# anuragranj/cc

Measured on AMD Instinct MI355X. Metric: train images/sec (832x256, 5-frame sample, 6-scale CC step), higher is better.
Workload: dtype f32; 1 GPU; full CC: DispResNet6+PoseNetB6+MaskNet6+Back2Future, all losses; per_gpu_batch=4, global_batch=4, height=256, width=832, scales=6, frames=5, parallelism=dp1, hipgraph=True, trained_nets=all, rccl_ranks=1, dead_occlusion_decoders_elided=False, net_streams=2, pipeline=per_network, grad_chunks=False, deterministic=True

## Files before the change

### cc_amd/csrc/wgrad_thin.hip

```cpp
#include <stdio.h>
#include <type_traits>
#include <stdlib.h>
#include "cc_common.h"
#include "conv_internal.h"
#include "cc_tools.h"

namespace {

typedef float f32x4 __attribute__((ext_vector_type(4)));

constexpr int THIN_NW = 4;

struct WT {
    const float* a; const float* x; float* ws;
    int B, M, AH, AW; long a_bs;
    int Cin, IH, IW; long x_bs;
    int R, nxc, units, upb, npb, ngc, ngt, swz;
};

template <int S, int SI, int PAD, int TR>
struct ThinCfg {
    static constexpr int PQ = (PAD + 3) / 4;
    static constexpr int IMAX = SI * 3 + S - 1 - PAD + 4 * PQ;
    static constexpr int NQ = IMAX / 4 + 1;
    static constexpr int TS = TR * S;
};

template <int S, int SI, int PAD, int TR, int DBG>
__device__ __forceinline__ void wgrad_thin_body(const WT& g, const int bx_, const int by_) {
    typedef ThinCfg<S, SI, PAD, TR> C;
    constexpr int PQ = C::PQ, NQ = C::NQ, TS = C::TS;
    __shared__ float red[TS * 256];
    const int lane = threadIdx.x & 63;
    const int wave = __builtin_amdgcn_readfirstlane((int)(threadIdx.x >> 6));
    const int i = lane & 15, k = lane >> 4;
    int combo = by_;
    const int tg = combo % g.ngt;
    combo /= g.ngt;
    const int cg = combo % g.ngc, mg = combo / g.ngc;
    const int r0 = tg * TR;
    const int m = mg * 16 + i, c = cg * 16 + i;
    const bool mok = m < g.M, cok = c < g.Cin;
    const float* __restrict__ abase = g.a + (long)(mok ? m : 0) * g.AH * g.AW;
    const float* __restrict__ xbase = g.x + (long)(cok ? c : 0) * g.IH * g.IW;

    f32x4 acc[TR][S];
#pragma unroll
    for (int tr = 0; tr < TR; tr++)
#pragma unroll
        for (int s = 0; s < S; s++) acc[tr][s] = (f32x4){0.f, 0.f, 0.f, 0.f};

    const int pb = (g.swz ? ((bx_ & 7) * (g.npb >> 3) + (bx_ >> 3)) : bx_);
    const int u0 = pb * g.upb;
    const int u1 = (u0 + g.upb < g.units) ? (u0 + g.upb) : g.units;

    constexpr int KEEP = (TR > SI) ? TR - SI : 0;
    float4 An;
    float4 Wn[TR][NQ], Wc[TR][NQ];
    auto issue = [&](auto T0, int b, int y, int xc, float4& A, float4 (&W)[TR][NQ]) {
        constexpr int t0 = decltype(T0)::value;
        const int x0 = xc * 16 + 4 * k;
        const int xa = (x0 < g.AW) ? x0 : 0;
        A = *(const float4*)(abase + (unsigned)(b * (int)g.a_bs + y * g.AW + xa));
        const unsigned xb = (unsigned)(b * (int)g.x_bs);
#pragma unroll
        for (int tr = t0; tr < TR; tr++) {
            int iy = y * SI + r0 + tr - PAD;
            iy = iy < 0 ? 0 : (iy >= g.IH ? g.IH - 1 : iy);
            const unsigned xr = xb + (unsigned)(iy * g.IW);
#pragma unroll
            for (int q = 0; q < NQ; q++) {
                int col = SI * x0 - 4 * PQ + 4 * q;
                col = (col < 0 || col >= g.IW) ? 0 : col;
                W[tr][q] = *(const float4*)(xbase + (xr + (unsigned)col));
            }
        }
    };

    const int ngx = (g.nxc + THIN_NW - 1) / THIN_NW;
    int u = u0;
    const int ue = u1;
    if (u < ue) {
        int nb, ny, nxcpos;
        {
            const int colu = u / g.AH;
            ny = u - colu * g.AH;
            nb = colu / ngx;
            nxcpos = (colu - nb * ngx) * THIN_NW + wave;
        }
        typedef std::integral_constant<int, 0> ALL;
        typedef std::integral_constant<int, KEEP> NEW;
        issue(ALL(), nb, ny, nxcpos, An, Wn);
        bool fresh = true;
        for (; u < ue; u++) {
            const float4 Ac = An;
            if (fresh) {
#pragma unroll
                for (int tr = 0; tr < TR; tr++)
#pragma unroll
                    for (int q = 0; q < NQ; q++) Wc[tr][q] = Wn[tr][q];
            } else {
#pragma unroll
                for (int tr = 0; tr < TR; tr++)
#pragma unroll
                    for (int q = 0; q < NQ; q++) Wc[tr][q] = (tr < KEEP) ? Wc[tr + (TR - KEEP)][q] : Wn[tr][q];
            }
            const int y = ny, xc = nxcpos;
            if (u + 1 < ue) {
                fresh = false;
                if (++ny == g.AH) {
                    ny = 0;
                    fresh = true;
                    nxcpos += THIN_NW;
                    if (nxcpos - wave >= g.nxc) { nxcpos = wave; nb++; }
                }
                if (DBG != 2) {
                    if (fresh) issue(ALL(), nb, ny, nxcpos, An, Wn);
                    else issue(NEW(), nb, ny, nxcpos, An, Wn);
                }
            }

            const int x0 = xc * 16 + 4 * k;
            const bool aok = mok && (x0 < g.AW);
            float a4[4];
            a4[0] = aok ? Ac.x : 0.f;
            a4[1] = aok ? Ac.y : 0.f;
            a4[2] = aok ? Ac.z : 0.f;
            a4[3] = aok ? Ac.w : 0.f;
#pragma unroll
            for (int tr = 0; tr < TR; tr++) {
                const int iy = y * SI + r0 + tr - PAD;
                const bool rok = cok && (r0 + tr < g.R) && iy >= 0 && iy < g.IH;
                float w[NQ * 4];
#pragma unroll
                for (int q = 0; q < NQ; q++) {
                    const int col = SI * x0 - 4 * PQ + 4 * q;
                    const bool ok = rok && col >= 0 && col < g.IW;
                    w[4 * q + 0] = ok ? Wc[tr][q].x : 0.f;
                    w[4 * q + 1] = ok ? Wc[tr][q].y : 0.f;
                    w[4 * q + 2] = ok ? Wc[tr][q].z : 0.f;
                    w[4 * q + 3] = ok ? Wc[tr][q].w : 0.f;
                }
                if (DBG == 1) {
#pragma unroll
                    for (int s = 0; s < S; s++)
#pragma unroll
                        for (int j = 0; j < 4; j++) acc[tr][s][j] += a4[j] * w[SI * j + s - PAD + 4 * PQ];
                    continue;
                }
#pragma unroll
                for (int j = 0; j < 4; j++)
#pragma unroll
                    for (int s = 0; s < S; s++)
                        acc[tr][s] = __builtin_amdgcn_mfma_f32_16x16x4f32(a4[j], w[SI * j + s - PAD + 4 * PQ], acc[tr][s], 0, 0, 0);
            }
        }
    }

#pragma unroll 1
    for (int wv = 0; wv < THIN_NW; wv++) {
        if (wave == wv) {
#pragma unroll
            for (int tr = 0; tr < TR; tr++)
#pragma unroll
                for (int s = 0; s < S; s++)
#pragma unroll
                    for (int r = 0; r < 4; r++) {
                        const int idx = ((tr * S + s) * 4 + r) * 64 + lane;
                        const float v = acc[tr][s][r];
                        red[idx] = (wv == 0) ? v : (red[idx] + v);
                    }
        }
        __syncthreads();
    }
    float* __restrict__ slab = g.ws + ((long)by_ * g.npb + pb) * (TS * 256);
    for (int e = threadIdx.x; e < TS * 256; e += 64 * THIN_NW) {
        const int t = e >> 8, mc = e & 255, mm = mc >> 4, cc_ = mc & 15;
        slab[e] = red[(t * 4 + (mm & 3)) * 64 + (mm >> 2) * 16 + cc_];
    }
}


template <int S, int SI, int PAD, int TR, int DBG = 0>
__global__ __launch_bounds__(64 * THIN_NW) void k_wgrad_thin(WT g) {
    wgrad_thin_body<S, SI, PAD, TR, DBG>(g, (int)blockIdx.x, (int)blockIdx.y);
}

constexpr int THIN_MAXP = 24;
struct WTM { WT p[THIN_MAXP]; int blk_end[THIN_MAXP]; int n; };
template <int S, int SI, int PAD, int TR>
__global__ __launch_bounds__(64 * THIN_NW) void k_wgrad_thin_multi(WTM a) {
    int k = 0, first = 0;
#pragma unroll 1
    for (int q = 0; q + 1 < a.n; q++)
        if ((int)blockIdx.x >= a.blk_end[q]) { k = q + 1; first = a.blk_end[q]; }
#if defined(__HIP_DEVICE_COMPILE__) && !defined(CC_HIPEMU)
    const WT& g = *(reinterpret_cast<const WT*>((const char*)__builtin_amdgcn_kernarg_segment_ptr() + offsetof(WTM, p)) + k);
#else
    const WT& g = a.p[k];
#endif
    const int b = (int)blockIdx.x - first;
    const int by = b / g.npb;
    wgrad_thin_body<S, SI, PAD, TR, 0>(g, b - by * g.npb, by);
}


int env_int(const char* name, int dflt) { return cctools::env_int(name, dflt); }

struct ThinPlan {
    bool ok;
    int kind, TR, ngm, ngc, ngt, nxc, units, upb, npb, TS;
    size_t ws_floats;
};

enum { K_3_1 = 0, K_3_2, K_7_2, K_7_1, K_1_1, K_5_2, K_4_2, K_1_2, K_NONE };

ThinPlan plan_thin(int B, int M, int AH, int AW, int Cin, int R, int S, int si) {
    ThinPlan p = {};
    p.kind = K_NONE;
    if (R != S || env_int("CC_NO_WGRAD_THIN", 0)) return p;
    if (S == 3 && si == 1) { p.kind = K_3_1; p.TR = 3; }
    else if (S == 3 && si == 2) { p.kind = K_3_2; p.TR = 3; }
    else if (S == 7 && si == 2) { p.kind = K_7_2; p.TR = 2; }
    else if (S == 7 && si == 1) { p.kind = K_7_1; p.TR = 2; }
    else if (S == 1 && si == 1) { p.kind = K_1_1; p.TR = 1; }
    else if (S == 5 && si == 2) { p.kind = K_5_2; p.TR = 3; }
    else if (S == 4 && si == 2) { p.kind = K_4_2; p.TR = 4; }
    else if (S == 1 && si == 2) { p.kind = K_1_2; p.TR = 1; }
    else return p;
    p.ngm = (M + 15) / 16;
    p.ngc = (Cin + 15) / 16;
    const long P = (long)B * AH * AW;
    if ((AW & 3) || p.ngm * p.ngc > env_int("CC_WGRAD_THIN_MAXCOMBO", 15) || P < env_int("CC_WGRAD_THIN_MINPIX", 8192) ||
        (S == 7 && Cin < 8)) return p;
    p.ngt = (R + p.TR - 1) / p.TR;
    p.TS = p.TR * S;
    p.nxc = (AW + 15) / 16;
    const long units = (long)B * AH * ((p.nxc + THIN_NW - 1) / THIN_NW);
    if (units > (1l << 30)) return p;
    p.units = (int)units;
    long npb = units / env_int("CC_WGRAD_THIN_UPB", 8);
    const long cap = env_int("CC_WGRAD_THIN_NPB", 256);
    npb = npb < 1 ? 1 : (npb > cap ? cap : npb);
    p.upb = (int)((units + npb - 1) / npb);
    p.npb = (p.units + p.upb - 1) / p.upb;
    if (p.npb >= 64) p.npb = ((p.npb + 7) / 8) * 8;
    p.ws_floats = (size_t)p.ngm * p.ngc * p.ngt * p.npb * p.TS * 256;
    p.ok = true;
    return p;
}

template <int S, int SI, int PAD, int TR>
void launch_thin(const WT& g, dim3 grid, hipStream_t s) {
    hipLaunchKernelGGL(HIP_KERNEL_NAME(k_wgrad_thin<S, SI, PAD, TR>), grid, dim3(64 * THIN_NW), 0, s, g);
}

template <int S, int SI, int PAD, int TR>
void launch_thin_multi(const WTM& m, unsigned blocks, hipStream_t s) {
    hipLaunchKernelGGL(HIP_KERNEL_NAME(k_wgrad_thin_multi<S, SI, PAD, TR>), dim3(blocks), dim3(64 * THIN_NW), 0, s, m);
}

constexpr int THIN_PARK_CAP = 96;
struct ThinParkedOne { WT g; int kind, ncombo; double gflop; };
struct ThinParked { bool on; int n; ThinParkedOne d[THIN_PARK_CAP]; };
thread_local ThinParked g_thin_parked = {};

void launch_thin_kind(int kind, const WT& g, dim3 grid, hipStream_t s) {
    switch (kind) {
        case K_3_1: launch_thin<3, 1, 1, 3>(g, grid, s); break;
        case K_3_2: launch_thin<3, 2, 1, 3>(g, grid, s); break;
        case K_7_2: launch_thin<7, 2, 3, 2>(g, grid, s); break;
        case K_7_1: launch_thin<7, 1, 3, 2>(g, grid, s); break;
        case K_1_1: launch_thin<1, 1, 0, 1>(g, grid, s); break;
        case K_5_2: launch_thin<5, 2, 2, 3>(g, grid, s); break;
        case K_1_2: launch_thin<1, 2, 0, 1>(g, grid, s); break;
        default: launch_thin<4, 2, 1, 4>(g, grid, s); break;
    }
}

void launch_thin_multi_kind(int kind, const WTM& m, unsigned blocks, hipStream_t s) {
    switch (kind) {
        case K_3_1: launch_thin_multi<3, 1, 1, 3>(m, blocks, s); break;
        case K_3_2: launch_thin_multi<3, 2, 1, 3>(m, blocks, s); break;
        case K_7_2: launch_thin_multi<7, 2, 3, 2>(m, blocks, s); break;
        case K_7_1: launch_thin_multi<7, 1, 3, 2>(m, blocks, s); break;
        case K_1_1: launch_thin_multi<1, 1, 0, 1>(m, blocks, s); break;
        case K_5_2: launch_thin_multi<5, 2, 2, 3>(m, blocks, s); break;
        case K_1_2: launch_thin_multi<1, 2, 0, 1>(m, blocks, s); break;
        default: launch_thin_multi<4, 2, 1, 4>(m, blocks, s); break;
    }
}

}

namespace ccint {

bool wgrad_thin_park(bool on) {
    const bool was = g_thin_parked.on;
    g_thin_parked.on = on && !env_int("CC_NO_WGRAD_THIN_LIST", 0);
    return was;
}

bool wgrad_thin_parking() { return g_thin_parked.on; }

double wgrad_thin_parked_gflop() {
    double gf = 0;
    for (int i = 0; i < g_thin_parked.n; i++) gf += g_thin_parked.d[i].gflop;
    return gf;
}

void wgrad_thin_flush(hipStream_t s) {
    ThinParked& P = g_thin_parked;
    for (int kind = 0; kind < K_NONE && P.n > 0; kind++) {
        int i = 0;
        while (i < P.n) {
            WTM m = {};
            long blk = 0;
            int last = -1;
            for (; i < P.n && m.n < THIN_MAXP; i++) {
                if (P.d[i].kind != kind) continue;
                const long nb = (long)P.d[i].g.npb * P.d[i].ncombo;
                if (m.n && blk + nb >= (1l << 31)) break;
                m.p[m.n] = P.d[i].g;
                blk += nb;
                m.blk_end[m.n] = (int)blk;
                m.n++;
                last = i;
            }
            if (!m.n) break;
            if (env_int("CC_WGRAD_THIN_TRACE", 0)) fprintf(stderr, "[wgrad_thin_multi] kind %d: %d problems, %ld workgroups\n", kind, m.n, blk);
            if (m.n == 1) launch_thin_kind(kind, P.d[last].g, dim3((unsigned)P.d[last].g.npb, (unsigned)P.d[last].ncombo), s);
            else launch_thin_multi_kind(kind, m, (unsigned)blk, s);
        }
    }
    P.n = 0;
}

size_t wgrad_thin_ws_floats(int B, int M, int AH, int AW, int Cin, int R, int S, int si) {
    const ThinPlan p = plan_thin(B, M, AH, AW, Cin, R, S, si);
    return p.ok ? p.ws_floats : 0;
}

bool wgrad_thin_launch(const float* a, const float* x, float* gw, float* ws, int B, int M, int AH, int AW, long a_bs, int Cin,
                       int IH, int IW, long x_bs, int R, int S, int si, int pad, long o_sm, long o_sc, int accumulate, hipStream_t s,
                       RedSink* sink) {
    const ThinPlan p = plan_thin(B, M, AH, AW, Cin, R, S, si);
    if (!p.ok || (IW & 3) || (a_bs & 3) || (x_bs & 3) || (((uintptr_t)a | (uintptr_t)x) & 15)) return false;
    if ((long)B * a_bs >= (1l << 31) || (long)B * x_bs >= (1l << 31)) return false;
    static const int want_pad[] = {1, 1, 3, 3, 0, 2, 1, 0};
    if (pad != want_pad[p.kind]) return false;
    WT g = {};
    g.a = a; g.x = x; g.ws = ws;
    g.B = B; g.M = M; g.AH = AH; g.AW = AW; g.a_bs = a_bs; g.Cin = Cin; g.IH = IH; g.IW = IW; g.x_bs = x_bs;
    g.R = R; g.nxc = p.nxc; g.units = p.units; g.upb = p.upb; g.npb = p.npb; g.ngc = p.ngc; g.ngt = p.ngt;
    g.swz = (p.npb % 8 == 0 && p.npb >= 64 && !env_int("CC_WGRAD_THIN_NOSWZ", 0)) ? 1 : 0;
    const int ncombo = p.ngm * p.ngc * p.ngt;
    if (env_int("CC_WGRAD_THIN_TRACE", 0))
        fprintf(stderr, "[wgrad_thin] kind %d M %d Cin %d A %dx%d X %dx%d npb %d upb %d combos %d\n", p.kind, M, Cin, AH, AW, IH, IW,
                p.npb, p.upb, ncombo);
    dim3 grid((unsigned)p.npb, (unsigned)ncombo);
    if (g_thin_parked.on && sink && g_thin_parked.n < THIN_PARK_CAP) {
        ThinParkedOne& d = g_thin_parked.d[g_thin_parked.n++];
        d.g = g; d.kind = p.kind; d.ncombo = ncombo;
        d.gflop = 2e-9 * B * AH * AW * (double)M * Cin * R * S;
        const long rdp[RD_LONGS] = {2, (long)ws, (long)gw, p.npb, accumulate, o_sm, o_sc, p.TS, S, p.TR, p.ngc, p.ngt, M, Cin, R, ncombo};
        (void)wgrad_reduce_emit(sink, rdp, 1, s);
        return true;
    }
    switch (p.kind) {
        case K_3_1: {
            const int dbg = env_int("CC_WGRAD_THIN_DBG", 0);
            if (dbg == 1) hipLaunchKernelGGL(HIP_KERNEL_NAME(k_wgrad_thin<3, 1, 1, 3, 1>), grid, dim3(64 * THIN_NW), 0, s, g);
            else if (dbg == 2) hipLaunchKernelGGL(HIP_KERNEL_NAME(k_wgrad_thin<3, 1, 1, 3, 2>), grid, dim3(64 * THIN_NW), 0, s, g);
            else launch_thin<3, 1, 1, 3>(g, grid, s);
            break;
        }
        case K_3_2: launch_thin<3, 2, 1, 3>(g, grid, s); break;
        case K_7_2: launch_thin<7, 2, 3, 2>(g, grid, s); break;
        case K_7_1: launch_thin<7, 1, 3, 2>(g, grid, s); break;
        case K_1_1: launch_thin<1, 1, 0, 1>(g, grid, s); break;
        case K_5_2: launch_thin<5, 2, 2, 3>(g, grid, s); break;
        case K_1_2: launch_thin<1, 2, 0, 1>(g, grid, s); break;
        default: launch_thin<4, 2, 1, 4>(g, grid, s); break;
    }
    const long rd[RD_LONGS] = {2, (long)ws, (long)gw, p.npb, accumulate, o_sm, o_sc, p.TS, S, p.TR, p.ngc, p.ngt, M, Cin, R, ncombo};
    (void)wgrad_reduce_emit(sink, rd, 1, s);
    return true;
}

void wgrad_thin_name(int B, int M, int AH, int AW, int Cin, int IH, int IW, int R, int S, int si, int pad, char* out, int cap) {
    out[0] = 0;
    const ThinPlan p = plan_thin(B, M, AH, AW, Cin, R, S, si);
    static const int want_pad[] = {1, 1, 3, 3, 0, 2, 1, 0};
    static const int tr[] = {3, 3, 2, 2, 1, 3, 4, 1};
    if (!p.ok || (IW & 3) || pad != want_pad[p.kind]) return;
    snprintf(out, cap, "k_wgrad_thin<%d, %d, %d, %d>", S, si, pad, tr[p.kind]);
}

}
```

Baseline: 251.7 images/s.

## Bundle multiple 16-wide M/C groups per workgroup in thin weight-gradient kernel

Lets each thin wgrad workgroup compute up to 2x2 output-channel/input-channel 16-wide groups. The loaded activation and input tiles are reused across several MFMA accumulators, and fewer workgroups are launched. By default bundling is on only for the 1x1 kernels (stride 1 and 2); other kinds keep 1x1 unless an env var is set. The cost is higher register pressure and serialized LDS reductions per bundled group, which can lower occupancy.

New measurement: 252.5 images/s, median of 6. No clear change (+0.3%).

```diff
diff --git a/cc_amd/csrc/wgrad_thin.hip b/cc_amd/csrc/wgrad_thin.hip
--- a/cc_amd/csrc/wgrad_thin.hip
+++ b/cc_amd/csrc/wgrad_thin.hip
@@ -16,6 +16,7 @@
     int B, M, AH, AW; long a_bs;
     int Cin, IH, IW; long x_bs;
     int R, nxc, units, upb, npb, ngc, ngt, swz;
+    int ngm, bm, bc, nbc;
 };
 
 template <int S, int SI, int PAD, int TR>
@@ -26,42 +27,55 @@
     static constexpr int TS = TR * S;
 };
 
-template <int S, int SI, int PAD, int TR, int DBG>
-__device__ __forceinline__ void wgrad_thin_body(const WT& g, const int bx_, const int by_) {
+template <int S, int SI, int PAD, int TR, int MG, int CG, int DBG>
+__device__ __forceinline__ void wgrad_thin_body(const WT& g, const int bx_, const int mg0, const int cg0, const int tg,
+                                                float* __restrict__ red) {
     typedef ThinCfg<S, SI, PAD, TR> C;
     constexpr int PQ = C::PQ, NQ = C::NQ, TS = C::TS;
-    __shared__ float red[TS * 256];
     const int lane = threadIdx.x & 63;
     const int wave = __builtin_amdgcn_readfirstlane((int)(threadIdx.x >> 6));
     const int i = lane & 15, k = lane >> 4;
-    int combo = by_;
-    const int tg = combo % g.ngt;
-    combo /= g.ngt;
-    const int cg = combo % g.ngc, mg = combo / g.ngc;
     const int r0 = tg * TR;
-    const int m = mg * 16 + i, c = cg * 16 + i;
-    const bool mok = m < g.M, cok = c < g.Cin;
-    const float* __restrict__ abase = g.a + (long)(mok ? m : 0) * g.AH * g.AW;
-    const float* __restrict__ xbase = g.x + (long)(cok ? c : 0) * g.IH * g.IW;
-
-    f32x4 acc[TR][S];
-#pragma unroll
-    for (int tr = 0; tr < TR; tr++)
-#pragma unroll
-        for (int s = 0; s < S; s++) acc[tr][s] = (f32x4){0.f, 0.f, 0.f, 0.f};
+    bool mok[MG], cok[CG];
+    const float* __restrict__ abase[MG];
+    const float* __restrict__ xbase[CG];
+#pragma unroll
+    for (int mi = 0; mi < MG; mi++) {
+        const int m = (mg0 + mi) * 16 + i;
+        mok[mi] = m < g.M;
+        abase[mi] = g.a + (long)(mok[mi] ? m : 0) * g.AH * g.AW;
+    }
+#pragma unroll
+    for (int ci = 0; ci < CG; ci++) {
+        const int c = (cg0 + ci) * 16 + i;
+        cok[ci] = c < g.Cin;
+        xbase[ci] = g.x + (long)(cok[ci] ? c : 0) * g.IH * g.IW;
+    }
+
+    f32x4 acc[MG][CG][TR][S];
+#pragma unroll
+    for (int mi = 0; mi < MG; mi++)
+#pragma unroll
+        for (int ci = 0; ci < CG; ci++)
+#pragma unroll
+            for (int tr = 0; tr < TR; tr++)
+#pragma unroll
+                for (int s = 0; s < S; s++) acc[mi][ci][tr][s] = (f32x4){0.f, 0.f, 0.f, 0.f};
 
     const int pb = (g.swz ? ((bx_ & 7) * (g.npb >> 3) + (bx_ >> 3)) : bx_);
     const int u0 = pb * g.upb;
     const int u1 = (u0 + g.upb < g.units) ? (u0 + g.upb) : g.units;
 
     constexpr int KEEP = (TR > SI) ? TR - SI : 0;
-    float4 An;
-    float4 Wn[TR][NQ], Wc[TR][NQ];
-    auto issue = [&](auto T0, int b, int y, int xc, float4& A, float4 (&W)[TR][NQ]) {
+    float4 An[MG];
+    float4 Wn[CG][TR][NQ], Wc[CG][TR][NQ];
+    auto issue = [&](auto T0, int b, int y, int xc, float4 (&A)[MG], float4 (&W)[CG][TR][NQ]) {
         constexpr int t0 = decltype(T0)::value;
         const int x0 = xc * 16 + 4 * k;
         const int xa = (x0 < g.AW) ? x0 : 0;
-        A = *(const float4*)(abase + (unsigned)(b * (int)g.a_bs + y * g.AW + xa));
+        const unsigned ao = (unsigned)(b * (int)g.a_bs + y * g.AW + xa);
+#pragma unroll
+        for (int mi = 0; mi < MG; mi++) A[mi] = *(const float4*)(abase[mi] + ao);
         const unsigned xb = (unsigned)(b * (int)g.x_bs);
 #pragma unroll
         for (int tr = t0; tr < TR; tr++) {
@@ -72,7 +86,8 @@
             for (int q = 0; q < NQ; q++) {
                 int col = SI * x0 - 4 * PQ + 4 * q;
                 col = (col < 0 || col >= g.IW) ? 0 : col;
-                W[tr][q] = *(const float4*)(xbase + (xr + (unsigned)col));
+#pragma unroll
+                for (int ci = 0; ci < CG; ci++) W[ci][tr][q] = *(const float4*)(xbase[ci] + (xr + (unsigned)col));
             }
         }
     };
@@ -93,17 +108,23 @@
         issue(ALL(), nb, ny, nxcpos, An, Wn);
         bool fresh = true;
         for (; u < ue; u++) {
-            const float4 Ac = An;
+            float4 Ac[MG];
+#pragma unroll
+            for (int mi = 0; mi < MG; mi++) Ac[mi] = An[mi];
             if (fresh) {
 #pragma unroll
-                for (int tr = 0; tr < TR; tr++)
-#pragma unroll
-                    for (int q = 0; q < NQ; q++) Wc[tr][q] = Wn[tr][q];
+                for (int ci = 0; ci < CG; ci++)
+#pragma unroll
+                    for (int tr = 0; tr < TR; tr++)
+#pragma unroll
+                        for (int q = 0; q < NQ; q++) Wc[ci][tr][q] = Wn[ci][tr][q];
             } else {
 #pragma unroll
-                for (int tr = 0; tr < TR; tr++)
-#pragma unroll
-                    for (int q = 0; q < NQ; q++) Wc[tr][q] = (tr < KEEP) ? Wc[tr + (TR - KEEP)][q] : Wn[tr][q];
+                for (int ci = 0; ci < CG; ci++)
+#pragma unroll
+                    for (int tr = 0; tr < TR; tr++)
+#pragma unroll
+                        for (int q = 0; q < NQ; q++) Wc[ci][tr][q] = (tr < KEEP) ? Wc[ci][tr + (TR - KEEP)][q] : Wn[ci][tr][q];
             }
             const int y = ny, xc = nxcpos;
             if (u + 1 < ue) {
@@ -121,75 +142,117 @@
             }
 
             const int x0 = xc * 16 + 4 * k;
-            const bool aok = mok && (x0 < g.AW);
-            float a4[4];
-            a4[0] = aok ? Ac.x : 0.f;
-            a4[1] = aok ? Ac.y : 0.f;
-            a4[2] = aok ? Ac.z : 0.f;
-            a4[3] = aok ? Ac.w : 0.f;
+            float a4[MG][4];
+#pragma unroll
+            for (int mi = 0; mi < MG; mi++) {
+                const bool aok = mok[mi] && (x0 < g.AW);
+                a4[mi][0] = aok ? Ac[mi].x : 0.f;
+                a4[mi][1] = aok ? Ac[mi].y : 0.f;
+                a4[mi][2] = aok ? Ac[mi].z : 0.f;
+                a4[mi][3] = aok ? Ac[mi].w : 0.f;
+            }
 #pragma unroll
             for (int tr = 0; tr < TR; tr++) {
                 const int iy = y * SI + r0 + tr - PAD;
-                const bool rok = cok && (r0 + tr < g.R) && iy >= 0 && iy < g.IH;
-                float w[NQ * 4];
+                const bool rok = (r0 + tr < g.R) && iy >= 0 && iy < g.IH;
+                float w[CG][NQ * 4];
 #pragma unroll
                 for (int q = 0; q < NQ; q++) {
                     const int col = SI * x0 - 4 * PQ + 4 * q;
-                    const bool ok = rok && col >= 0 && col < g.IW;
-                    w[4 * q + 0] = ok ? Wc[tr][q].x : 0.f;
-                    w[4 * q + 1] = ok ? Wc[tr][q].y : 0.f;
-                    w[4 * q + 2] = ok ? Wc[tr][q].z : 0.f;
-                    w[4 * q + 3] = ok ? Wc[tr][q].w : 0.f;
+                    const bool qok = rok && col >= 0 && col < g.IW;
+#pragma unroll
+                    for (int ci = 0; ci < CG; ci++) {
+                        const bool ok = qok && cok[ci];
+                        w[ci][4 * q + 0] = ok ? Wc[ci][tr][q].x : 0.f;
+                        w[ci][4 * q + 1] = ok ? Wc[ci][tr][q].y : 0.f;
+                        w[ci][4 * q + 2] = ok ? Wc[ci][tr][q].z : 0.f;
+                        w[ci][4 * q + 3] = ok ? Wc[ci][tr][q].w : 0.f;
+                    }
                 }
                 if (DBG == 1) {
 #pragma unroll
                     for (int s = 0; s < S; s++)
 #pragma unroll
-                        for (int j = 0; j < 4; j++) acc[tr][s][j] += a4[j] * w[SI * j + s - PAD + 4 * PQ];
+                        for (int j = 0; j < 4; j++) acc[0][0][tr][s][j] += a4[0][j] * w[0][SI * j + s - PAD + 4 * PQ];
                     continue;
                 }
 #pragma unroll
                 for (int j = 0; j < 4; j++)
 #pragma unroll
                     for (int s = 0; s < S; s++)
-                        acc[tr][s] = __builtin_amdgcn_mfma_f32_16x16x4f32(a4[j], w[SI * j + s - PAD + 4 * PQ], acc[tr][s], 0, 0, 0);
+#pragma unroll
+                        for (int mi = 0; mi < MG; mi++)
+#pragma unroll
+                            for (int ci = 0; ci < CG; ci++)
+                                acc[mi][ci][tr][s] = __builtin_amdgcn_mfma_f32_16x16x4f32(a4[mi][j], w[ci][SI * j + s - PAD + 4 * PQ],
+                                                                                          acc[mi][ci][tr][s], 0, 0, 0);
             }
         }
     }
 
+#pragma unroll
+    for (int mi = 0; mi < MG; mi++)
+#pragma unroll
+        for (int ci = 0; ci < CG; ci++) {
+            if (mi + ci) __syncthreads();
 #pragma unroll 1
-    for (int wv = 0; wv < THIN_NW; wv++) {
-        if (wave == wv) {
-#pragma unroll
-            for (int tr = 0; tr < TR; tr++)
-#pragma unroll
-                for (int s = 0; s < S; s++)
-#pragma unroll
-                    for (int r = 0; r < 4; r++) {
-                        const int idx = ((tr * S + s) * 4 + r) * 64 + lane;
-                        const float v = acc[tr][s][r];
-                        red[idx] = (wv == 0) ? v : (red[idx] + v);
-                    }
+            for (int wv = 0; wv < THIN_NW; wv++) {
+                if (wave == wv) {
+#pragma unroll
+                    for (int tr = 0; tr < TR; tr++)
+#pragma unroll
+                        for (int s = 0; s < S; s++)
+#pragma unroll
+                            for (int r = 0; r < 4; r++) {
+                                const int idx = ((tr * S + s) * 4 + r) * 64 + lane;
+                                const float v = acc[mi][ci][tr][s][r];
+                                red[idx] = (wv == 0) ? v : (red[idx] + v);
+                            }
+                }
+                __syncthreads();
+            }
+            const int combo = ((mg0 + mi) * g.ngc + (cg0 + ci)) * g.ngt + tg;
+            float* __restrict__ slab = g.ws + ((long)combo * g.npb + pb) * (TS * 256);
+            for (int e = threadIdx.x; e < TS * 256; e += 64 * THIN_NW) {
+                const int t = e >> 8, mc = e & 255, mm = mc >> 4, cc_ = mc & 15;
+                slab[e] = red[(t * 4 + (mm & 3)) * 64 + (mm >> 2) * 16 + cc_];
+            }
         }
-        __syncthreads();
-    }
-    float* __restrict__ slab = g.ws + ((long)by_ * g.npb + pb) * (TS * 256);
-    for (int e = threadIdx.x; e < TS * 256; e += 64 * THIN_NW) {
-        const int t = e >> 8, mc = e & 255, mm = mc >> 4, cc_ = mc & 15;
-        slab[e] = red[(t * 4 + (mm & 3)) * 64 + (mm >> 2) * 16 + cc_];
-    }
-}
-
-
-template <int S, int SI, int PAD, int TR, int DBG = 0>
+}
+
+template <int S, int SI, int PAD, int TR, int MGX, int CGX, int DBG>
+__device__ __forceinline__ void wgrad_thin_bundle(const WT& g, const int bx_, const int by_, float* __restrict__ red) {
+    int bu = by_;
+    const int tg = bu % g.ngt;
+    bu /= g.ngt;
+    const int cb = bu % g.nbc, mb = bu / g.nbc;
+    const int mg0 = mb * g.bm, cg0 = cb * g.bc;
+    const bool m2 = MGX > 1 && g.bm > 1 && mg0 + 1 < g.ngm;
+    const bool c2 = CGX > 1 && g.bc > 1 && cg0 + 1 < g.ngc;
+    if constexpr (MGX > 1 && CGX > 1) {
+        if (m2 && c2) { wgrad_thin_body<S, SI, PAD, TR, 2, 2, DBG>(g, bx_, mg0, cg0, tg, red); return; }
+    }
+    if constexpr (MGX > 1) {
+        if (m2) { wgrad_thin_body<S, SI, PAD, TR, 2, 1, DBG>(g, bx_, mg0, cg0, tg, red); return; }
+    }
+    if constexpr (CGX > 1) {
+        if (c2) { wgrad_thin_body<S, SI, PAD, TR, 1, 2, DBG>(g, bx_, mg0, cg0, tg, red); return; }
+    }
+    wgrad_thin_body<S, SI, PAD, TR, 1, 1, DBG>(g, bx_, mg0, cg0, tg, red);
+}
+
+
+template <int S, int SI, int PAD, int TR, int MGX = 1, int CGX = 1, int DBG = 0>
 __global__ __launch_bounds__(64 * THIN_NW) void k_wgrad_thin(WT g) {
-    wgrad_thin_body<S, SI, PAD, TR, DBG>(g, (int)blockIdx.x, (int)blockIdx.y);
+    __shared__ float red[ThinCfg<S, SI, PAD, TR>::TS * 256];
+    wgrad_thin_bundle<S, SI, PAD, TR, MGX, CGX, DBG>(g, (int)blockIdx.x, (int)blockIdx.y, red);
 }
 
 constexpr int THIN_MAXP = 24;
 struct WTM { WT p[THIN_MAXP]; int blk_end[THIN_MAXP]; int n; };
-template <int S, int SI, int PAD, int TR>
+template <int S, int SI, int PAD, int TR, int MGX, int CGX>
 __global__ __launch_bounds__(64 * THIN_NW) void k_wgrad_thin_multi(WTM a) {
+    __shared__ float red[ThinCfg<S, SI, PAD, TR>::TS * 256];
     int k = 0, first = 0;
 #pragma unroll 1
     for (int q = 0; q + 1 < a.n; q++)
@@ -201,7 +264,7 @@
 #endif
     const int b = (int)blockIdx.x - first;
     const int by = b / g.npb;
-    wgrad_thin_body<S, SI, PAD, TR, 0>(g, b - by * g.npb, by);
+    wgrad_thin_bundle<S, SI, PAD, TR, MGX, CGX, 0>(g, b - by * g.npb, by, red);
 }
 
 
@@ -250,45 +313,58 @@
     return p;
 }
 
-template <int S, int SI, int PAD, int TR>
-void launch_thin(const WT& g, dim3 grid, hipStream_t s) {
-    hipLaunchKernelGGL(HIP_KERNEL_NAME(k_wgrad_thin<S, SI, PAD, TR>), grid, dim3(64 * THIN_NW), 0, s, g);
-}
-
-template <int S, int SI, int PAD, int TR>
-void launch_thin_multi(const WTM& m, unsigned blocks, hipStream_t s) {
-    hipLaunchKernelGGL(HIP_KERNEL_NAME(k_wgrad_thin_multi<S, SI, PAD, TR>), dim3(blocks), dim3(64 * THIN_NW), 0, s, m);
+struct ThinBundle { int bm, bc; };
+constexpr ThinBundle THIN_MAXB[K_NONE] = {{2, 2}, {2, 2}, {2, 2}, {2, 2}, {2, 2}, {2, 2}, {2, 1}, {2, 2}};
+constexpr ThinBundle THIN_SHIP[K_NONE] = {{1, 1}, {1, 1}, {1, 1}, {1, 1}, {2, 2}, {1, 1}, {1, 1}, {2, 2}};
+
+ThinBundle thin_bundle(const ThinPlan& p) {
+    const int mode = env_int("CC_WGRAD_THIN_GROUPS", 0);
+    ThinBundle b = mode >= 2 ? THIN_MAXB[p.kind] : mode == 1 ? ThinBundle{1, 1} : THIN_SHIP[p.kind];
+    b.bm = b.bm < p.ngm ? b.bm : p.ngm;
+    b.bc = b.bc < p.ngc ? b.bc : p.ngc;
+    return b;
+}
+
+template <int S, int SI, int PAD, int TR, int MGX, int CGX>
+void launch_thin(bool big, const WT& g, dim3 grid, hipStream_t s) {
+    if (big) hipLaunchKernelGGL(HIP_KERNEL_NAME(k_wgrad_thin<S, SI, PAD, TR, MGX, CGX>), grid, dim3(64 * THIN_NW), 0, s, g);
+    else hipLaunchKernelGGL(HIP_KERNEL_NAME(k_wgrad_thin<S, SI, PAD, TR>), grid, dim3(64 * THIN_NW), 0, s, g);
+}
+
+template <int S, int SI, int PAD, int TR, int MGX, int CGX>
+void launch_thin_multi(bool big, const WTM& m, unsigned blocks, hipStream_t s) {
+    if (big) hipLaunchKernelGGL(HIP_KERNEL_NAME(k_wgrad_thin_multi<S, SI, PAD, TR, MGX, CGX>), dim3(blocks), dim3(64 * THIN_NW), 0, s, m);
+    else hipLaunchKernelGGL(HIP_KERNEL_NAME(k_wgrad_thin_multi<S, SI, PAD, TR, 1, 1>), dim3(blocks), dim3(64 * THIN_NW), 0, s, m);
 }
 
 constexpr int THIN_PARK_CAP = 96;
-struct ThinParkedOne { WT g; int kind, ncombo; double gflop; };
+struct ThinParkedOne { WT g; int kind, nbundle; double gflop; };
 struct ThinParked { bool on; int n; ThinParkedOne d[THIN_PARK_CAP]; };
 thread_local ThinParked g_thin_parked = {};
 
-void launch_thin_kind(int kind, const WT& g, dim3 grid, hipStream_t s) {
-    switch (kind) {
-        case K_3_1: launch_thin<3, 1, 1, 3>(g, grid, s); break;
-        case K_3_2: launch_thin<3, 2, 1, 3>(g, grid, s); break;
-        case K_7_2: launch_thin<7, 2, 3, 2>(g, grid, s); break;
-        case K_7_1: launch_thin<7, 1, 3, 2>(g, grid, s); break;
-        case K_1_1: launch_thin<1, 1, 0, 1>(g, grid, s); break;
-        case K_5_2: launch_thin<5, 2, 2, 3>(g, grid, s); break;
-        case K_1_2: launch_thin<1, 2, 0, 1>(g, grid, s); break;
-        default: launch_thin<4, 2, 1, 4>(g, grid, s); break;
-    }
-}
-
-void launch_thin_multi_kind(int kind, const WTM& m, unsigned blocks, hipStream_t s) {
-    switch (kind) {
-        case K_3_1: launch_thin_multi<3, 1, 1, 3>(m, blocks, s); break;
-        case K_3_2: launch_thin_multi<3, 2, 1, 3>(m, blocks, s); break;
-        case K_7_2: launch_thin_multi<7, 2, 3, 2>(m, blocks, s); break;
-        case K_7_1: launch_thin_multi<7, 1, 3, 2>(m, blocks, s); break;
-        case K_1_1: launch_thin_multi<1, 1, 0, 1>(m, blocks, s); break;
-        case K_5_2: launch_thin_multi<5, 2, 2, 3>(m, blocks, s); break;
-        case K_1_2: launch_thin_multi<1, 2, 0, 1>(m, blocks, s); break;
-        default: launch_thin_multi<4, 2, 1, 4>(m, blocks, s); break;
-    }
+bool thin_big(int kind, const WT& g) { return THIN_SHIP[kind].bm * THIN_SHIP[kind].bc > 1 || g.bm * g.bc > 1; }
+
+#ifdef CC_TOOLS
+#define THIN_B(mg, cg) mg, cg
+#else
+#define THIN_B(mg, cg) 1, 1
+#endif
+#define THIN_KINDS(F, ...)                                                \
+    switch (kind) {                                                       \
+        case K_3_1: F<3, 1, 1, 3, THIN_B(2, 2)>(__VA_ARGS__); break;      \
+        case K_3_2: F<3, 2, 1, 3, THIN_B(2, 2)>(__VA_ARGS__); break;      \
+        case K_7_2: F<7, 2, 3, 2, THIN_B(2, 2)>(__VA_ARGS__); break;      \
+        case K_7_1: F<7, 1, 3, 2, THIN_B(2, 2)>(__VA_ARGS__); break;      \
+        case K_1_1: F<1, 1, 0, 1, 2, 2>(__VA_ARGS__); break;              \
+        case K_5_2: F<5, 2, 2, 3, THIN_B(2, 2)>(__VA_ARGS__); break;      \
+        case K_1_2: F<1, 2, 0, 1, 2, 2>(__VA_ARGS__); break;              \
+        default: F<4, 2, 1, 4, THIN_B(2, 1)>(__VA_ARGS__); break;         \
+    }
+
+void launch_thin_kind(int kind, const WT& g, dim3 grid, hipStream_t s) { THIN_KINDS(launch_thin, thin_big(kind, g), g, grid, s) }
+
+void launch_thin_multi_kind(int kind, bool big, const WTM& m, unsigned blocks, hipStream_t s) {
+    THIN_KINDS(launch_thin_multi, big, m, blocks, s)
 }
 
 }
@@ -311,15 +387,17 @@
 
 void wgrad_thin_flush(hipStream_t s) {
     ThinParked& P = g_thin_parked;
-    for (int kind = 0; kind < K_NONE && P.n > 0; kind++) {
+    for (int kb = 0; kb < 2 * K_NONE && P.n > 0; kb++) {
+        const int kind = kb >> 1;
+        const bool big = kb & 1;
         int i = 0;
         while (i < P.n) {
             WTM m = {};
             long blk = 0;
             int last = -1;
             for (; i < P.n && m.n < THIN_MAXP; i++) {
-                if (P.d[i].kind != kind) continue;
-                const long nb = (long)P.d[i].g.npb * P.d[i].ncombo;
+                if (P.d[i].kind != kind || thin_big(kind, P.d[i].g) != big) continue;
+                const long nb = (long)P.d[i].g.npb * P.d[i].nbundle;
                 if (m.n && blk + nb >= (1l << 31)) break;
                 m.p[m.n] = P.d[i].g;
                 blk += nb;
@@ -328,9 +406,9 @@
                 last = i;
             }
             if (!m.n) break;
-            if (env_int("CC_WGRAD_THIN_TRACE", 0)) fprintf(stderr, "[wgrad_thin_multi] kind %d: %d problems, %ld workgroups\n", kind, m.n, blk);
-            if (m.n == 1) launch_thin_kind(kind, P.d[last].g, dim3((unsigned)P.d[last].g.npb, (unsigned)P.d[last].ncombo), s);
-            else launch_thin_multi_kind(kind, m, (unsigned)blk, s);
+            if (env_int("CC_WGRAD_THIN_TRACE", 0)) fprintf(stderr, "[wgrad_thin_multi] kind %d%s: %d problems, %ld workgroups\n", kind, big ? " bundled" : "", m.n, blk);
+            if (m.n == 1) launch_thin_kind(kind, P.d[last].g, dim3((unsigned)P.d[last].g.npb, (unsigned)P.d[last].nbundle), s);
+            else launch_thin_multi_kind(kind, big, m, (unsigned)blk, s);
         }
     }
     P.n = 0;
@@ -355,34 +433,25 @@
     g.R = R; g.nxc = p.nxc; g.units = p.units; g.upb = p.upb; g.npb = p.npb; g.ngc = p.ngc; g.ngt = p.ngt;
     g.swz = (p.npb % 8 == 0 && p.npb >= 64 && !env_int("CC_WGRAD_THIN_NOSWZ", 0)) ? 1 : 0;
     const int ncombo = p.ngm * p.ngc * p.ngt;
+    const int dbg = p.kind == K_3_1 ? env_int("CC_WGRAD_THIN_DBG", 0) : 0;
+    const ThinBundle bu = dbg ? ThinBundle{1, 1} : thin_bundle(p);
+    g.ngm = p.ngm; g.bm = bu.bm; g.bc = bu.bc; g.nbc = (p.ngc + bu.bc - 1) / bu.bc;
+    const int nbundle = ((p.ngm + bu.bm - 1) / bu.bm) * g.nbc * p.ngt;
     if (env_int("CC_WGRAD_THIN_TRACE", 0))
-        fprintf(stderr, "[wgrad_thin] kind %d M %d Cin %d A %dx%d X %dx%d npb %d upb %d combos %d\n", p.kind, M, Cin, AH, AW, IH, IW,
-                p.npb, p.upb, ncombo);
-    dim3 grid((unsigned)p.npb, (unsigned)ncombo);
+        fprintf(stderr, "[wgrad_thin] kind %d M %d Cin %d A %dx%d X %dx%d npb %d upb %d combos %d bundles %d of %dx%d\n", p.kind, M, Cin,
+                AH, AW, IH, IW, p.npb, p.upb, ncombo, nbundle, bu.bm, bu.bc);
+    dim3 grid((unsigned)p.npb, (unsigned)nbundle);
     if (g_thin_parked.on && sink && g_thin_parked.n < THIN_PARK_CAP) {
         ThinParkedOne& d = g_thin_parked.d[g_thin_parked.n++];
-        d.g = g; d.kind = p.kind; d.ncombo = ncombo;
+        d.g = g; d.kind = p.kind; d.nbundle = nbundle;
         d.gflop = 2e-9 * B * AH * AW * (double)M * Cin * R * S;
         const long rdp[RD_LONGS] = {2, (long)ws, (long)gw, p.npb, accumulate, o_sm, o_sc, p.TS, S, p.TR, p.ngc, p.ngt, M, Cin, R, ncombo};
         (void)wgrad_reduce_emit(sink, rdp, 1, s);
         return true;
     }
-    switch (p.kind) {
-        case K_3_1: {
-            const int dbg = env_int("CC_WGRAD_THIN_DBG", 0);
-            if (dbg == 1) hipLaunchKernelGGL(HIP_KERNEL_NAME(k_wgrad_thin<3, 1, 1, 3, 1>), grid, dim3(64 * THIN_NW), 0, s, g);
-            else if (dbg == 2) hipLaunchKernelGGL(HIP_KERNEL_NAME(k_wgrad_thin<3, 1, 1, 3, 2>), grid, dim3(64 * THIN_NW), 0, s, g);
-            else launch_thin<3, 1, 1, 3>(g, grid, s);
-            break;
-        }
-        case K_3_2: launch_thin<3, 2, 1, 3>(g, grid, s); break;
-        case K_7_2: launch_thin<7, 2, 3, 2>(g, grid, s); break;
-        case K_7_1: launch_thin<7, 1, 3, 2>(g, grid, s); break;
-        case K_1_1: launch_thin<1, 1, 0, 1>(g, grid, s); break;
-        case K_5_2: launch_thin<5, 2, 2, 3>(g, grid, s); break;
-        case K_1_2: launch_thin<1, 2, 0, 1>(g, grid, s); break;
-        default: launch_thin<4, 2, 1, 4>(g, grid, s); break;
-    }
+    if (dbg == 1) hipLaunchKernelGGL(HIP_KERNEL_NAME(k_wgrad_thin<3, 1, 1, 3, 1, 1, 1>), grid, dim3(64 * THIN_NW), 0, s, g);
+    else if (dbg == 2) hipLaunchKernelGGL(HIP_KERNEL_NAME(k_wgrad_thin<3, 1, 1, 3, 1, 1, 2>), grid, dim3(64 * THIN_NW), 0, s, g);
+    else launch_thin_kind(p.kind, g, grid, s);
     const long rd[RD_LONGS] = {2, (long)ws, (long)gw, p.npb, accumulate, o_sm, o_sc, p.TS, S, p.TR, p.ngc, p.ngt, M, Cin, R, ncombo};
     (void)wgrad_reduce_emit(sink, rd, 1, s);
     return true;
```
